# tesseract-robotics/trajopt

Hardware: NVIDIA B200
Metric: converged trajectories/sec (7-DOF x 30 wp, batch 1024) (higher is better)
Workload: dtype f64

## Files before the change

### trajopt_b200/csrc/qp_cta_kernel.cuh

```cuda
#pragma once
#include "device_types.cuh"
#include "joint_terms.cuh"

namespace tb200 {

#ifdef TB200_PROFILE
static __device__ unsigned long long g_prof[16];
#define PROF_T0() const long long prof_t0_ = clock64()
#define PROF_ADD(slot) do { if (q.tid == 0) atomicAdd(&g_prof[slot], (unsigned long long)(clock64() - prof_t0_)); } while (0)
#else
#define PROF_T0()
#define PROF_ADD(slot)
#endif
#if defined(TB200_PROFILE) && defined(TB200_PROFILE_CHECK)
#define PROF_CHK_T0() long long pc_ = clock64()
#define PROF_CHK(slot) do { const long long n_ = clock64(); if (q.tid == 0) atomicAdd(&g_prof[slot], (unsigned long long)(n_ - pc_)); pc_ = n_; } while (0)
#else
#define PROF_CHK_T0()
#define PROF_CHK(slot)
#endif

constexpr int kQpThreads = 256;
constexpr int kQpThreadsC = 256;
constexpr double kOsqpInf = 1e30;
// ... 100 lines not shown
  return s;
}

enum RowF {
  R_C = 0, R_W,
  R_E, R_DA0, R_DA1, R_EA0, R_EA1,
  R_U0, R_U1, R_B0, R_B1, R_LO, R_UP, R_QA0, R_QA1, R_RHO,
  R_XA0, R_XA1, R_Z, R_Y, R_ZA0, R_ZA1, R_YA0, R_YA1,
  R_RA0, R_RA1, R_COEF, R_WR, R_G0, R_G1, R_DEN, R_WRR,
  R_IDEN, R_IWRR,
  R_DY, R_DYA0, R_DYA1, R_DXA0, R_DXA1,
  R_PW, R_PWA0, R_PWA1, R_PB, R_PY, R_PYA0, R_PYA1, R_PX0, R_PX1,
  R_MV,
  R_NF
};
__host__ __device__ inline int qp_row_stride(int CN) { return 3 * CN + R_NF; }

struct SmVec {
  int off;
  __device__ __forceinline__ double* ptr() const {
    extern __shared__ double sm[];
    return sm + off;
  }
  __device__ __forceinline__ double& operator[](int i) const { return ptr()[i]; }
  __device__ __forceinline__ operator double*() const { return ptr(); }
  __device__ __forceinline__ SmVec& operator=(double* p) {
    extern __shared__ double sm[];
    off = static_cast<int>(p - sm);
    return *this;
  }
};

struct QpCtx {
  int N, Np, nb, M, T, D, CN, RS, tid, nrows;
  double *SA, *SLM, *SU;
  SmVec beta, x, zb, yb, v1, w, qs, lbs, ubs, tmp, red, flag;
  int* colptr;
  SmVec Dz, v2;
  double* rows;
  double* soa;
  double* smbase;
  int rows_smem;
  int* rints;
  const int* colent;
  const double* Pband;
  const int* band_offs;
  int n_band;
  double* scratch;
  int pinv;
  PinvPlan pl;
  double* pi_g;
  double* z_stash;
  double c, cinv, rho, rho_eq, sigma, alpha;
  __device__ __forceinline__ double* R(int r) const { return rows + static_cast<size_t>(r) * RS; }
  __device__ __forceinline__ double* F(int r) const { return rows + static_cast<size_t>(r) * RS + 2 * CN; }
  __device__ __forceinline__ const int* I(int r) const { return rints + static_cast<size_t>(r) * RI_NINTS; }
};

__device__ __forceinline__ double warp_max_norm(double v) {
  v = (v != v) ? 0.0 : v;
  const unsigned hi = static_cast<unsigned>(__double2hiint(v)) & 0x7fffffffu, lo = static_cast<unsigned>(__double2loint(v));
  const unsigned mh = __reduce_max_sync(0xffffffffu, hi);
  const unsigned ml = __reduce_max_sync(0xffffffffu, hi == mh ? lo : 0u);
  return __hiloint2double(static_cast<int>(mh), static_cast<int>(ml));
}
template <int NQ, unsigned SUM_MASK>
__device__ __forceinline__ void block_reduce(const QpCtx& q, double (&vals)[NQ]) {
  static_assert(NQ <= 16, "red area too small");
  extern __shared__ double sm[];
  double* const red = sm + (q.red - q.smbase);
  const int lane = q.tid & 31, wid = q.tid >> 5;
  __syncwarp();
#pragma unroll
  for (int k = 0; k < NQ; ++k) {
    double v = vals[k];
    if ((SUM_MASK >> k) & 1u) {
#pragma unroll
      for (int off = 16; off > 0; off >>= 1) v += __shfl_xor_sync(0xffffffffu, v, off);
    } else {
      v = warp_max_norm(v);
    }
    vals[k] = v;
  }
  if (lane == 0) {
#pragma unroll
    for (int k = 0; k < NQ; ++k) red[k * 8 + wid] = vals[k];
  }
  __syncthreads();
#pragma unroll
  for (int k = 0; k < NQ; ++k) {
    if ((SUM_MASK >> k) & 1u) {
      double acc = red[k * 8];
#pragma unroll
      for (int w = 1; w < kQpThreads / 32; ++w) acc += red[k * 8 + w];
      vals[k] = acc;
    } else {
      vals[k] = warp_max_norm(red[k * 8 + (lane & 7)]);
    }
  }
  __syncthreads();
}

struct SysW {
  bool polish;
  double sig, rho_aux;
};

__device__ __forceinline__ int row_var(const int* I, int k) {
  return I[RI_BASE] + min(k, I[RI_CNT] - 1) * I[RI_STRIDE];
}

template <int NB>
__device__ __forceinline__ void load_row(double (&a)[NB], const double* src) {
  const double2* s2 = reinterpret_cast<const double2*>(src);
#pragma unroll
  for (int k = 0; k < NB / 2; ++k) {
    const double2 v = s2[k];
    a[2 * k] = v.x;
    a[2 * k + 1] = v.y;
  }
}
template <int NB>
__device__ __forceinline__ void store_row(double* dst, const double (&a)[NB]) {
  double2* d2 = reinterpret_cast<double2*>(dst);
#pragma unroll
  for (int k = 0; k < NB / 2; ++k) d2[k] = make_double2(a[2 * k], a[2 * k + 1]);
}
template <int NB>
__device__ __forceinline__ void row_times_mat(double (&out)[NB], const double (&x)[NB], const double* Y) {
#pragma unroll
  for (int k = 0; k < NB; ++k) {
    double y[NB];
    load_row<NB>(y, Y + k * NB);
#pragma unroll
    for (int j = 0; j < NB; ++j) out[j] += x[k] * y[j];
  }
}
template <int NB>
__device__ __forceinline__ void row_times_matT(double (&out)[NB], const double (&x)[NB], const double* Y) {
#pragma unroll
  for (int j = 0; j < NB; ++j) {
    double y[NB];
    load_row<NB>(y, Y + j * NB);
    double a0 = 0.0, a1 = 0.0;
#pragma unroll
    for (int k = 0; k < NB; k += 2) {
      a0 += x[k] * y[k];
      a1 += x[k + 1] * y[k + 1];
    }
    out[j] += a0 + a1;
  }
}
template <int NB>
__device__ inline bool bcr_factor(const QpCtx& q) {
  constexpr int BLK = NB * NB, G = kQpThreads / 2;
  constexpr int CH1 = kQpThreads / NB, CH2 = G / NB;
  const int M = q.M, tid = q.tid;
  const int grp = tid >= G, gt = tid - (grp ? G : 0);
  int bad = 0;
  for (int l = 0; (1 << l) - 1 < M; ++l) {
    const int s = 1 << l, first = s - 1, sh = l + 1;
    const int nE = (M + s) >> sh, nS = M >> sh;
    for (int e0 = 0; e0 < nE; e0 += CH1) {
      const int nc = (nE - e0 < CH1) ? nE - e0 : CH1;
      const bool act = tid < nc * NB;
      const int e = act ? tid / NB : 0, i = tid % NB;
      double* A = q.SA + (first + ((e0 + e) << sh)) * BLK + i * NB;
      double a[NB];
      load_row<NB>(a, A);
#pragma unroll
      for (int k = 0; k < NB; ++k) {
        double* prow = q.tmp + (k & 1) * (CH1 * NB) + e * NB;
        if (act && i == k) {
          const double piv = a[k];
          if (!(piv > 0.0)) bad = 1;
          const double ip = 1.0 / piv;
#pragma unroll
          for (int j = 0; j < NB; ++j) a[j] = (j == k) ? ip : a[j] * ip;
          store_row<NB>(prow, a);
        }
        __syncthreads();
        if (act && i != k) {
          double pr[NB];
          load_row<NB>(pr, prow);
          const double f = a[k];
#pragma unroll
          for (int j = 0; j < NB; ++j) a[j] = (j == k) ? -f * pr[k] : a[j] - f * pr[j];
        }
      }
      if (act) store_row<NB>(A, a);
    }
    __syncthreads();
    for (int e0 = 0; e0 < nE; e0 += CH2) {
      const int nc = (nE - e0 < CH2) ? nE - e0 : CH2;
      const bool act = gt < nc * NB;
      const int e = e0 + (act ? gt / NB : 0), i = gt % NB;
      const int p = first + (e << sh);
      const double* Ai = q.SA + p * BLK;
      if (act && grp == 0 && p + s < M) {
        double x[NB], out[NB];
        load_row<NB>(x, q.SLM + (p + s) * BLK + i * NB);
#pragma unroll
        for (int j = 0; j < NB; ++j) out[j] = 0.0;
        row_times_mat<NB>(out, x, Ai);
        store_row<NB>(q.SU + p * BLK + i * NB, out);
      }
      if (act && grp == 1 && p - s >= 0) {
        double x[NB], out[NB];
        const double* L = q.SLM + p * BLK + i;
#pragma unroll
        for (int k = 0; k < NB; ++k) x[k] = L[k * NB];
#pragma unroll
        for (int j = 0; j < NB; ++j) out[j] = 0.0;
        row_times_mat<NB>(out, x, Ai);
        store_row<NB>(q.SU + (p - s) * BLK + i * NB, out);
      }
    }
    __syncthreads();
    for (int e0 = 0; e0 < nS; e0 += CH2) {
      const int nc = (nS - e0 < CH2) ? nS - e0 : CH2;
      const bool act = gt < nc * NB;
      const int e = e0 + (act ? gt / NB : 0), i = gt % NB;
      const int j = first + s + (e << sh), p = j - s;
      double keep[NB];
#pragma unroll
      for (int c = 0; c < NB; ++c) keep[c] = 0.0;
      if (act && grp == 0) {
        double x[NB], t1[NB];
        load_row<NB>(x, q.SU + p * BLK + i * NB);
#pragma unroll
        for (int c = 0; c < NB; ++c) t1[c] = 0.0;
        row_times_matT<NB>(t1, x, q.SLM + j * BLK);
        if (p - s >= 0) row_times_mat<NB>(keep, x, q.SLM + p * BLK);
        double arow[NB];
        load_row<NB>(arow, q.SA + j * BLK + i * NB);
#pragma unroll
        for (int c = 0; c < NB; ++c) arow[c] -= t1[c];
        store_row<NB>(q.SA + j * BLK + i * NB, arow);
      }
      if (act && grp == 1 && j + s < M) {
        double x[NB];
        load_row<NB>(x, q.SU + j * BLK + i * NB);
        row_times_mat<NB>(keep, x, q.SLM + (j + s) * BLK);
      }
      __syncthreads();
      if (act && grp == 0) {
#pragma unroll
        for (int c = 0; c < NB; ++c) keep[c] = -keep[c];
        store_row<NB>(q.SLM + j * BLK + i * NB, keep);
      }
      if (act && grp == 1 && j + s < M) {
        double arow[NB];
        load_row<NB>(arow, q.SA + j * BLK + i * NB);
#pragma unroll
        for (int c = 0; c < NB; ++c) arow[c] -= keep[c];
        store_row<NB>(q.SA + j * BLK + i * NB, arow);
      }
    }
    __syncthreads();
    for (int t = tid; t < nE * BLK; t += kQpThreads) {
      const int e = t / BLK, r = t % BLK;
      const int p = first + (e << sh);
      if (p - s >= 0) q.SLM[p * BLK + r] = q.SU[(p - s) * BLK + r];
    }
    __syncthreads();
  }
  if (tid == 0) q.flag[0] = 0.0;
  __syncthreads();
  if (bad) q.flag[0] = 1.0;
  __syncthreads();
  const bool ok = q.flag[0] == 0.0;
  __syncthreads();
  return ok;
}

template <int NB>
__device__ __forceinline__ double dot_row(const double* __restrict__ m, const double* __restrict__ v) {
  const double2* m2 = reinterpret_cast<const double2*>(m);
  const double2* v2 = reinterpret_cast<const double2*>(v);
  double a0 = 0.0, a1 = 0.0;
#pragma unroll
  for (int k = 0; k < NB / 2; ++k) {
    const double2 mm = m2[k], vv = v2[k];
    a0 += mm.x * vv.x;
    a1 += mm.y * vv.y;
  }
  return a0 + a1;
}
template <int NB>
__device__ inline void bcr_solve(const QpCtx& q, double* v, double* w) {
  constexpr int BLK = NB * NB, H = NB / 2;
  const int M = q.M, tid = q.tid, side = tid & 1, task0 = tid >> 1;
  __syncthreads();
  int l = 0;
  for (; (2 << l) - 1 < M; ++l) {
    const int s = 1 << l, sh = l + 1, nS = M >> sh;
    for (int tb = 0; tb < nS * NB; tb += kQpThreads / 2) {
      if (tb + ((tid & ~31) >> 1) >= nS * NB) continue;
      const int task = tb + task0;
      const int e = task / NB, r = task % NB;
      const bool act = e < nS;
      const int j = 2 * s - 1 + ((act ? e : 0) << sh);
      const int pb = side ? j + s : j - s;
      const bool valid = act && pb < M;
      const int pbc = valid ? pb : j - s;
      const double* mat = (side ? q.SLM : q.SU) + pbc * BLK + r * NB;
      double a = dot_row<NB>(mat, v + pbc * NB);
      a = valid ? a : 0.0;
      const double o = __shfl_xor_sync(0xffffffffu, a, 1);
      if (act && side == 0) v[j * NB + r] -= a + o;
    }
    __syncthreads();
  }
  for (; l >= 0; --l) {
    const int s = 1 << l, first = s - 1, sh = l + 1;
    if (first >= M) continue;
    const int nE = (M + s) >> sh;
    for (int tb = 0; tb < nE * NB; tb += kQpThreads / 2) {
      if (tb + ((tid & ~31) >> 1) >= nE * NB) continue;
      const int task = tb + task0;
      const int e = task / NB, r = task % NB;
      const bool act = e < nE;
      const int p = first + ((act ? e : 0) << sh);
      const bool hasl = p - s >= 0, hasr = p + s < M;
      const double* X = (side ? q.SU : q.SA) + p * BLK + r;
      const double* y = side ? w + (hasr ? p + s : 0) * NB : v + p * NB;
      const double* Um = q.SLM + p * BLK + (side ? H * NB : 0) + r;
      const double* wl = w + (hasl ? p - s : 0) * NB + (side ? H : 0);
      double a0 = 0.0, a1 = 0.0, a2 = 0.0;
#pragma unroll
      for (int k = 0; k < NB; k += 2) {
        a0 += X[k * NB] * y[k];
        a1 += X[(k + 1) * NB] * y[k + 1];
      }
#pragma unroll
      for (int k = 0; k < H; ++k) a2 += Um[k * NB] * wl[k];
      const double dx = a0 + a1;
      const double acc = (side ? (hasr ? -dx : 0.0) : dx) - (hasl ? a2 : 0.0);
      const double o = __shfl_xor_sync(0xffffffffu, acc, 1);
      if (act && side == 0) w[p * NB + r] = acc + o;
    }
    __syncthreads();
  }
}

struct SolveRoles {
  int n_fwd, n_lvl;
  int f0_warps, b0_warps;
  int f0_vec, f0_dst, b0_y, b0_wl, b0_dst;
  int fu_level, fu_vec, fu_dst, bu_level, bu_y, bu_wl, bu_dst;
  bool f0_valid, f0_store, b0_store, b0_hasl, b0_hasr, b0_yw;
  bool fu_valid, fu_store, bu_store, bu_hasl, bu_hasr, bu_yw;
  int fu_mat, bu_X, bu_Um, f0_mat, b0_X, b0_Um;
};
template <int NB>
__device__ inline SolveRoles solve_roles(const QpCtx& q) {
  SolveRoles R{};
  const int M = q.M, tid = q.tid;
  int nf = 0;
  while ((2 << nf) - 1 < M) ++nf;
  int nl = 0;
  while ((1 << nl) - 1 < M) ++nl;
  R.n_fwd = nf;
  R.n_lvl = nl;
  constexpr int BLK = NB * NB;
  const int oSA = static_cast<int>(q.SA - q.smbase), oSLM = static_cast<int>(q.SLM - q.smbase), oSU = static_cast<int>(q.SU - q.smbase);
  auto fwd_role = [&](int l, int u, int& vec, int& dst, bool& valid, bool& store) {
    const int s = 1 << l, sh = l + 1, nS = M >> sh;
    const int task = u >> 1, side = u & 1, e = task / NB, r = task % NB;
    const bool act = e < nS;
    const int j = 2 * s - 1 + ((act ? e : 0) << sh);
    const int pb = side ? j + s : j - s;
    valid = act && pb < M;
    vec = (valid ? pb : j - s) * NB;
    dst = j * NB + r;
    store = act && side == 0;
    (l > 0 ? R.fu_mat : R.f0_mat) = (side ? oSLM : oSU) + (valid ? pb : j - s) * BLK + r * NB;
  };
  auto bwd_role = [&](int l, int u, int& y, int& wl, int& dst, bool& store, bool& hasl, bool& hasr, bool& yw) {
    const int s = 1 << l, first = s - 1, sh = l + 1, nE = (M + s) >> sh;
    const int task = u >> 1, side = u & 1, e = task / NB, r = task % NB;
    const bool act = e < nE;
    const int p = first + ((act ? e : 0) << sh);
    hasl = p - s >= 0;
    hasr = p + s < M;
    yw = side;
    y = side ? (hasr ? p + s : 0) * NB : p * NB;
    wl = (hasl ? p - s : 0) * NB + (side ? NB / 2 : 0);
    dst = p * NB + r;
    store = act && side == 0;
    (l > 0 ? R.bu_X : R.b0_X) = (side ? oSU : oSA) + p * BLK + r;
    (l > 0 ? R.bu_Um : R.b0_Um) = oSLM + p * BLK + (side ? (NB / 2) * NB : 0) + r;
  };
  fwd_role(0, tid, R.f0_vec, R.f0_dst, R.f0_valid, R.f0_store);
  R.f0_warps = (2 * (M >> 1) * NB + 31) & ~31;
  bwd_role(0, tid, R.b0_y, R.b0_wl, R.b0_dst, R.b0_store, R.b0_hasl, R.b0_hasr, R.b0_yw);
  R.b0_warps = (2 * ((M + 1) >> 1) * NB + 31) & ~31;
  R.fu_level = -1;
  R.bu_level = -1;
  int off = 0;
  for (int l = 1; l < nf; ++l) {
    const int cnt = 2 * (M >> (l + 1)) * NB;
    if (tid >= off && tid < off + cnt) {
      R.fu_level = l;
      fwd_role(l, tid - off, R.fu_vec, R.fu_dst, R.fu_valid, R.fu_store);
    }
    off += cnt;
  }
  off = 0;
  for (int l = 1; l < nl; ++l) {
    const int cnt = 2 * ((M + (1 << l)) >> (l + 1)) * NB;
    if (tid >= off && tid < off + cnt) {
      R.bu_level = l;
      bwd_role(l, tid - off, R.bu_y, R.bu_wl, R.bu_dst, R.bu_store, R.bu_hasl, R.bu_hasr, R.bu_yw);
    }
    off += cnt;
  }
  return R;
}
__host__ __device__ inline bool solve_roles_fit(int M, int NB) {
  int f = 0, b = 0;
  for (int l = 1; (2 << l) - 1 < M; ++l) f += 2 * (M >> (l + 1)) * NB;
  for (int l = 1; (1 << l) - 1 < M; ++l) b += 2 * ((M + (1 << l)) >> (l + 1)) * NB;
  return f <= kQpThreads && b <= kQpThreads && 2 * ((M + 1) >> 1) * NB <= kQpThreads;
}
template <int NB>
// ... 259 lines not shown
  __syncthreads();
  for (int l = 1; l < R.n_fwd; ++l) {
    const bool mine = R.fu_level == l;
    if (__any_sync(0xffffffffu, mine)) {
      double a = reg_fwd_task<NB>(mFU, v + (mine ? R.fu_vec : 0));
      a = (mine && R.fu_valid) ? a : 0.0;
      const double o = __shfl_xor_sync(0xffffffffu, a, 1);
      if (mine && R.fu_store) v[R.fu_dst] -= a + o;
    }
    __syncthreads();
  }
  for (int l = R.n_lvl - 1; l >= 1; --l) {
    const bool mine = R.bu_level == l;
    if (__any_sync(0xffffffffu, mine)) {
      double acc = reg_bwd_task<NB>(mBU, (R.bu_yw ? w : v) + (mine ? R.bu_y : 0), w + (mine ? R.bu_wl : 0), R.bu_yw,
                                    R.bu_hasl, R.bu_hasr);
      acc = mine ? acc : 0.0;
      const double o = __shfl_xor_sync(0xffffffffu, acc, 1);
      if (mine && R.bu_store) w[R.bu_dst] = acc + o;
    }
    __syncthreads();
  }
  if (wbase < R.b0_warps) {
    const double acc = reg_bwd_task<NB>(mB0, (side ? w : v) + R.b0_y, w + R.b0_wl, side, R.b0_hasl, R.b0_hasr);
    const double o = __shfl_xor_sync(0xffffffffu, acc, 1);
    if (R.b0_store) w[R.b0_dst] = acc + o;
  }
  __syncthreads();
}

template <int NB>
__device__ __forceinline__ void bcr_solve_hyb(const int tid, const SolveRoles& R, const double (&mF0)[NB],
                                              const double (&mB0)[NB + NB / 2], const double* sm_base, double* v, double* w) {
  const int wbase = tid & ~31;
  const bool side = tid & 1;
  __syncthreads();
  if (wbase < R.f0_warps) {
#ifndef TB200_HYB_F0_REGS
    double a = bcr_fwd_task<NB>(sm_base + R.f0_mat, v + R.f0_vec);
#else
    double a = reg_fwd_task<NB>(mF0, v + R.f0_vec);
#endif
    a = R.f0_valid ? a : 0.0;
    const double o = __shfl_xor_sync(0xffffffffu, a, 1);
    if (R.f0_store) v[R.f0_dst] -= a + o;
  }
  __syncthreads();
  for (int l = 1; l < R.n_fwd; ++l) {
    const bool mine = R.fu_level == l;
    if (__any_sync(0xffffffffu, mine)) {
      double a = bcr_fwd_task<NB>(sm_base + (mine ? R.fu_mat : 0), v + (mine ? R.fu_vec : 0));
      a = (mine && R.fu_valid) ? a : 0.0;
      const double o = __shfl_xor_sync(0xffffffffu, a, 1);
      if (mine && R.fu_store) v[R.fu_dst] -= a + o;
    }
    __syncthreads();
  }
  for (int l = R.n_lvl - 1; l >= 1; --l) {
    const bool mine = R.bu_level == l;
    if (__any_sync(0xffffffffu, mine)) {
      double acc = bcr_bwd_task<NB>(sm_base + (mine ? R.bu_X : 0), sm_base + (mine ? R.bu_Um : 0),
                                    (R.bu_yw ? w : v) + (mine ? R.bu_y : 0), w + (mine ? R.bu_wl : 0), R.bu_yw, R.bu_hasl,
                                    R.bu_hasr);
      acc = mine ? acc : 0.0;
      const double o = __shfl_xor_sync(0xffffffffu, acc, 1);
      if (mine && R.bu_store) w[R.bu_dst] = acc + o;
    }
    __syncthreads();
  }
  if (wbase < R.b0_warps) {
    const double acc = reg_bwd_task<NB>(mB0, (side ? w : v) + R.b0_y, w + R.b0_wl, side, R.b0_hasl, R.b0_hasr);
    const double o = __shfl_xor_sync(0xffffffffu, acc, 1);
    if (R.b0_store) w[R.b0_dst] = acc + o;
  }
  __syncthreads();
}

template <int NB>
__device__ __forceinline__ void p_matvec(const QpCtx& q, const double* in, double* out) {
  extern __shared__ double sm[];
  constexpr int HB = NB, W = HB + 1;
  const int N = q.N, Np = q.Np, nbo = q.n_band;
  const double* const Pb = q.Pband;
  const double* const Dz = sm + (q.Dz - q.smbase);
  const double* const vin = sm + (in - q.smbase);
  double* const vout = sm + (out - q.smbase);
  const int* const offs = q.band_offs;
  const double cc = q.c;
  for (int i = q.tid; i < Np; i += kQpThreads) {
    double s = 0.0;
    if (i < N) {
      for (int t0 = 0; t0 < nbo; t0 += 4) {
        double v[4];
#pragma unroll
        for (int u = 0; u < 4; ++u) {
          const int k = (t0 + u < nbo) ? offs[t0 + u] : -1;
          v[u] = (k >= 0 && k <= i) ? (Pb[i * W + k] * Dz[i - k]) * vin[i - k] : 0.0;
        }
        s += v[0]; s += v[1]; s += v[2]; s += v[3];
      }
      for (int t0 = 0; t0 < nbo; t0 += 4) {
        double v[4];
#pragma unroll
        for (int u = 0; u < 4; ++u) {
          const int k = (t0 + u < nbo) ? offs[t0 + u] : -1;
          v[u] = (k >= 1 && i + k < N) ? (Pb[(i + k) * W + k] * Dz[i + k]) * vin[i + k] : 0.0;
        }
        s += v[0]; s += v[1]; s += v[2]; s += v[3];
      }
      s *= cc * Dz[i];
    }
    vout[i] = s;
  }
  __syncthreads();
}

__device__ inline void rows_prepare_weights(const QpCtx& q, const SysW& w) {
  for (int r = q.tid; r < q.nrows; r += kQpThreads) {
    double* F = q.F(r);
    const int naux = q.I(r)[RI_AUX];
    const double Wr = w.polish ? fabs(F[R_PW]) : ((F[R_RHO] != 0.0) ? q.rho_eq : q.rho);
    const double wa0 = w.polish ? fabs(F[R_PWA0]) : w.rho_aux;
    const double wa1 = w.polish ? fabs(F[R_PWA1]) : w.rho_aux;
    const double g0 = (naux >= 1) ? w.sig + wa0 * F[R_B0] * F[R_B0] : 1.0;
    const double g1 = (naux == 2) ? w.sig + wa1 * F[R_B1] * F[R_B1] : 1.0;
    const double den = g0 * g1 + Wr * (F[R_U0] * F[R_U0] * g1 + F[R_U1] * F[R_U1] * g0);
    F[R_WRR] = Wr;
    F[R_G0] = g0;
    F[R_G1] = g1;
    F[R_DEN] = den;
    F[R_IDEN] = 1.0 / den;
    F[R_IWRR] = (Wr != 0.0) ? 1.0 / Wr : 0.0;
    F[R_WR] = Wr * g0 * g1 / den;
  }
  __syncthreads();
}
__device__ __forceinline__ double xbound_weight(const QpCtx& q, const SysW& w, int j) {
  const double adm = (q.ubs[j] - q.lbs[j] < kRhoTol) ? q.rho_eq : q.rho;
  return w.polish ? fabs(q.zb[j]) : adm;
}

__device__ __forceinline__ double pivot_rcp(const double x) {
  double r;
  asm("rcp.approx.ftz.f64 %0, %1;" : "=d"(r) : "d"(x));
  double e = fma(-x, r, 1.0);
  r = fma(r, e, r);
  e = fma(-x, r, 1.0);
  r = fma(r, e, r);
  e = fma(-x, r, 1.0);
  return fma(r, e, r);
}
template <int QN>
__device__ __forceinline__ bool gj_rows(double (&a)[QN], double diag, const bool active, const int mat, const int row,
                                        const int n, const int n_max, double* tmp, const int nmat) {
  constexpr int BS = QN + 2;
  double* const csv = tmp + 2 * nmat * BS + mat * QN;
  bool bad = false;
  double pv_mine = pivot_rcp(diag), my_cs = 1.0, rs = 1.0, inv_rs = 1.0;
#pragma unroll 1
  for (int k = 0; k < n_max; ++k) {
    double* buf = tmp + ((k & 1) * nmat + mat) * BS;
    const bool piv = active && row == k;
    if (piv) {
      bad |= !(diag > 0.0);
#pragma unroll
      for (int j = 0; j < QN; j += 2) *reinterpret_cast<double2*>(buf + j) = make_double2(a[j], a[j + 1]);
      buf[k] = 0.0;
      buf[QN] = pv_mine;
      my_cs = -pv_mine;
      csv[k] = my_cs;
      rs = pv_mine;
      inv_rs = diag;
      diag = pv_mine;
    }
    __syncthreads();
    if (active && k < n && !piv) {
      const double tr = buf[row];
      const bool ahead = row > k;
      const double f = ahead ? tr : -tr * my_cs;
      const double g = f * buf[QN];
      diag = ahead ? diag - g * f : diag + g * f;
      const double gs = g * inv_rs;
#pragma unroll
      for (int j = 0; j < QN; j += 2) {
        const double2 t = *reinterpret_cast<const double2*>(buf + j);
        a[j] -= gs * t.x;
        a[j + 1] -= gs * t.y;
      }
      if (ahead) pv_mine = pivot_rcp(diag);
    }
  }
  if (active) {
#pragma unroll
    for (int j = 0; j < QN; ++j) a[j] = (j == row) ? diag : ((j < n) ? a[j] * (rs * csv[j]) : 0.0);
  }
  return bad;
}

template <int NB>
__device__ inline bool pinv_factor(const QpCtx& q) {
  constexpr int QN = 3 * NB, blk = NB * NB;
  static_assert(QN % 2 == 0, "pivot rows move as double2");
  extern __shared__ double sm[];
  const int tid = q.tid, M = q.M, Np = q.Np;
  const int PR = q.pl.PR, nS = q.pl.nS, Ns = q.pl.Ns, ZS = q.pl.ZS, WS = q.pl.WS, SS = q.pl.SS;
  double* const fbase = sm + (q.SA - q.smbase);
  const double* const SA = fbase;
  const double* const SLM = sm + (q.SLM - q.smbase);
  double* const Z = fbase + q.pl.zo;
  double* const W = fbase + q.pl.wo;
  double* const S = fbase + q.pl.so;
  double* const tmp = q.tmp.ptr();
  const int nparts = (M + 3) / 4;
  bool bad = false;
#ifdef TB200_PROFILE
  long long pf_ = clock64();
#define PROF_PF(slot) do { const long long n_ = clock64(); if (tid == 0) atomicAdd(&g_prof[slot], (unsigned long long)(n_ - pf_)); pf_ = n_; } while (0)
#else
#define PROF_PF(slot)
#endif
  {
    const bool prow = tid < PR;
    const int p = prow ? tid / QN : 0, lr = prow ? tid % QN : 0;
    const int npb = (M - 4 * p) < 3 ? (M - 4 * p) : 3;
    const int kb = lr / NB, r = lr % NB, gb = 4 * p + kb;
    double a[QN];
#pragma unroll
    for (int j = 0; j < QN; ++j) {
      const int cb = j / NB, c = j % NB;
      double v = 0.0;
      if (prow && cb < npb) {
        if (cb == kb) v = SA[gb * blk + r * NB + c];
        else if (cb == kb - 1) v = SLM[gb * blk + r * NB + c];
        else if (cb == kb + 1) v = SLM[(gb + 1) * blk + c * NB + r];
      }
      a[j] = v;
    }
    PROF_PF(0);
    const double dg = prow ? SA[gb * blk + r * NB + r] : 1.0;
    bad |= gj_rows<QN>(a, dg, prow, p, lr, npb * NB, (M < 3 ? M : 3) * NB, tmp, nparts);
    PROF_PF(4);
    if (prow) {
#pragma unroll
      for (int j = 0; j < QN; ++j) q.pi_g[tid * QN + j] = a[j];
      const bool has_l = p > 0, has_r = 4 * p + 3 < M;
#pragma unroll 2
      for (int j = 0; j < NB; ++j) {
        double wl = 0.0, wr = 0.0;
        if (has_l) {
#pragma unroll
          for (int c = 0; c < NB; ++c) wl += a[c] * SLM[(4 * p) * blk + c * NB + j];
        }
        if (has_r) {
#pragma unroll
          for (int c = 0; c < NB; ++c) wr += a[2 * NB + c] * SLM[(4 * p + 3) * blk + j * NB + c];
        }
        W[tid * WS + j] = wl;
        W[tid * WS + NB + j] = wr;
      }
    }
  }
  __syncthreads();
  for (int e = tid; e < nS * nS; e += kQpThreads) {
    const int ra = e / nS, ca = e % nS, sa = ra / NB, i = ra % NB, sb = ca / NB, j = ca % NB;
    double v = 0.0;
    if (sa == sb || sb == sa + 1 || sb == sa - 1) {
      const bool use_l = sb <= sa, use_r = sb >= sa && 4 * sa + 4 < M;
      const double* cl = SLM + (4 * sa + 3) * blk + i * NB;
      const double* wl = W + (sa * QN + 2 * NB) * WS + (sb == sa ? NB : 0) + j;
      const double* cr = SLM + (4 * sa + 4) * blk + i;
      const double* wr = W + ((sa + 1) * QN) * WS + (sb == sa ? 0 : NB) + j;
      double s0 = 0.0, s1 = 0.0, s2 = 0.0, s3 = 0.0;
      if (use_l) {
#pragma unroll
        for (int rr = 0; rr < NB; rr += 2) {
          s0 += cl[rr] * wl[rr * WS];
          s1 += cl[rr + 1] * wl[(rr + 1) * WS];
        }
      }
      if (use_r) {
#pragma unroll
        for (int rr = 0; rr < NB; rr += 2) {
          s2 += cr[rr * NB] * wr[rr * WS];
          s3 += cr[(rr + 1) * NB] * wr[(rr + 1) * WS];
        }
      }
      v = ((sa == sb) ? SA[(4 * sa + 3) * blk + i * NB + j] : 0.0) - ((s0 + s1) + (s2 + s3));
    }
    S[ra * SS + ca] = v;
  }
  __syncthreads();
  PROF_PF(14);
  {
    const bool srow = tid < nS;
    double a[QN];
#pragma unroll
    for (int j = 0; j < QN; ++j) a[j] = (srow && j < nS) ? S[tid * SS + j] : 0.0;
    const double dg = srow ? S[tid * SS + tid] : 1.0;
    bad |= gj_rows<QN>(a, dg, srow, 0, tid, nS, nS, tmp, 1);
    if (srow) {
#pragma unroll
      for (int j = 0; j < QN; ++j)
        if (j < nS) S[tid * SS + j] = a[j];
    }
  }
  __syncthreads();
  PROF_PF(15);
  if (tid < Np) {
    const int col = tid, cb = col / NB, c = col % NB, p = cb / 4;
    if (cb % 4 == 3) {
      for (int sr = 0; sr < nS; ++sr) Z[sr * ZS + col] = S[sr * SS + p * NB + c];
    } else {
      const bool has_l = p > 0, has_r = 4 * p + 3 < M;
      const double* wrow = W + (p * QN + (cb % 4) * NB + c) * WS;
      double wv[2 * NB];
#pragma unroll
      for (int t = 0; t < 2 * NB; ++t) wv[t] = wrow[t];
      const double* sl = S + (has_l ? (p - 1) * NB : 0);
      const double* sr_ = S + (has_r ? p * NB : 0);
#pragma unroll 2
      for (int sr = 0; sr < nS; ++sr) {
        double s0 = 0.0, s1 = 0.0, s2 = 0.0, s3 = 0.0;
#pragma unroll
        for (int t = 0; t < NB; t += 2) {
          s0 += sl[sr * SS + t] * wv[t];
          s1 += sl[sr * SS + t + 1] * wv[t + 1];
          s2 += sr_[sr * SS + t] * wv[NB + t];
          s3 += sr_[sr * SS + t + 1] * wv[NB + t + 1];
        }
        Z[sr * ZS + col] = -((s0 + s1) + (s2 + s3));
      }
    }
  }
  (void)Ns;
  const bool ok = !__syncthreads_or(bad ? 1 : 0);
  PROF_PF(9);
  return ok;
}

template <int NB, bool PINV>
__device__ __noinline__ bool assemble_factor(const QpCtx& q, const SysW& w) {
  PROF_T0();
  rows_prepare_weights(q, w);
  constexpr int nb = NB, blk = NB * NB;
  const int N = q.N, HB = 2 * q.D, PW = HB + 1, CN = q.CN;
  for (int t = q.tid; t < q.M * blk; t += kQpThreads) {
    q.SA[t] = 0.0;
    q.SLM[t] = 0.0;
  }
  __syncthreads();
  for (int i = q.tid; i < q.Np; i += kQpThreads) {
    const int p = i / nb, r = i % nb;
    double* Arow = q.SA + static_cast<size_t>(p) * blk + r * nb;
    double* Lrow = q.SLM + static_cast<size_t>(p) * blk + r * nb;
    if (i >= N) {
      Arow[r] = 1.0;
      continue;
    }
    auto add = [&](int k, double val) {
      if (k <= r) Arow[r - k] += val;
      else Lrow[nb + r - k] += val;
    };
    for (int t = 0; t < q.n_band; ++t) {
      const int k = q.band_offs[t];
      if (k <= i) add(k, q.c * q.Dz[i] * q.Pband[i * PW + k] * q.Dz[i - k]);
    }
    add(0, w.sig + xbound_weight(q, w, i) * q.beta[i] * q.beta[i]);
    for (int e = q.colptr[i]; e < q.colptr[i + 1]; ++e) {
      const int ent = q.colent[e], rw = ent >> 5, k = ent & 31;
      const double* R = q.R(rw);
      const double wr = R[2 * CN + R_WR];
      if (wr == 0.0) continue;
      const int stride = q.I(rw)[RI_STRIDE];
      const double* as = R + CN;
      const double ai = wr * as[k];
      for (int k2 = 0; k2 <= k; ++k2) add((k - k2) * stride, ai * as[k2]);
    }
  }
  __syncthreads();
  for (int t = q.tid; t < q.M * blk; t += kQpThreads) {
    const int p = t / blk, i = (t % blk) / nb, j = t % nb;
    if (j > i) q.SA[static_cast<size_t>(p) * blk + i * nb + j] = q.SA[static_cast<size_t>(p) * blk + j * nb + i];
  }
  __syncthreads();
  PROF_ADD(10);
  bool ok;
  {
    PROF_T0();
    if constexpr (PINV) ok = pinv_factor<NB>(q);
    else ok = bcr_factor<NB>(q);
    PROF_ADD(11);
  }
  return ok;
}

struct QpOut {
  int status, iters, polish;
  double rho;
  double pri_res, dua_res, pol_pri, pol_dua, c;
  int pol_factor_ok, rho_updates, rounds;
};

template <int CN, class Base>
__device__ __forceinline__ void scatter_columns(const QpCtx& q, Base base) {
  for (int i = q.tid; i < q.Np; i += kQpThreads) {
    double s = 0.0;
    if (i < q.N) {
      s = base(i);
      for (int e = q.colptr[i]; e < q.colptr[i + 1]; ++e) {
        const int ent = q.colent[e], r = ent >> 5, k = ent & 31;
        const double* R = q.R(r);
        s += R[CN + k] * R[2 * CN + R_COEF];
      }
    }
    q.v1[i] = s;
  }
  __syncthreads();
}
template <int CN>
__device__ __forceinline__ double row_dot(const QpCtx& q, const double* R, const int* I, const double* v) {
  double z = 0.0;
  const int base = I[RI_BASE], stride = I[RI_STRIDE], last = I[RI_CNT] - 1;
#pragma unroll
  for (int k = 0; k < CN; ++k) z += R[CN + k] * v[base + min(k, last) * stride];
  return z;
}
__device__ __forceinline__ void row_backsub(const double* F, double zeta, double& a0, double& a1) {
  const double Wr = F[R_WRR], ra0 = F[R_RA0], ra1 = F[R_RA1], u0 = F[R_U0], u1 = F[R_U1];
  const double iden = F[R_IDEN];
  a0 = (F[R_G1] * (ra0 - Wr * u0 * zeta) + Wr * u1 * (u1 * ra0 - u0 * ra1)) * iden;
  a1 = (F[R_G0] * (ra1 - Wr * u1 * zeta) + Wr * u0 * (u0 * ra1 - u1 * ra0)) * iden;
}
__device__ __forceinline__ double row_reduce_coef(const double* F, double ra0, double ra1, double zcoef) {
  return zcoef - F[R_WRR] * (F[R_U0] * ra0 * F[R_G1] + F[R_U1] * ra1 * F[R_G0]) * F[R_IDEN];
}

template <int NB, int PAIR, bool REG>
__device__ __noinline__ void admm_block(const QpCtx& q, const double rho_aux, const int n_iter, const int keep_last) {
  constexpr int CNc = PAIR ? ((NB > 3) ? NB : 3) : ((NB / 2 > 3) ? NB / 2 : 3);
  constexpr int RNB = REG ? NB : 2;
  const int N = q.N, tid = q.tid;
  double* const dxs = q.scratch;
  double* const dyb = q.scratch + q.Np;
  SolveRoles roles{};
  double mF0[RNB], mB0[RNB + RNB / 2], mFU[RNB], mBU[RNB + RNB / 2];
  if constexpr (REG) {
    roles = solve_roles<NB>(q);
    load_fwd_row<NB>(q, 0, tid, mF0);
    load_bwd_row<NB>(q, 0, tid, mB0);
    int off = 0;
    for (int l = 1; l < roles.n_fwd; ++l) {
      const int cnt = 2 * (q.M >> (l + 1)) * NB;
// ... 1752 lines not shown
```

Before: 1485.

## Use warp-per-block BCR factorization and named barriers in pinv Gauss-Jordan

Adds a warp-level block cyclic reduction factor path for NB<=16, where each warp factors one diagonal block with __syncwarp instead of CTA-wide barriers. The pinv partition Gauss-Jordan now gives each partition two warps and syncs them with per-partition named barriers, so independent partitions do not wait on each other. The loop bound drops to each partition's own size, and the reciprocal pivot is computed only for the next pivot row. The change risks named-barrier ID limits, a reduced thread count when nparts*64 exceeds the block, and lower parallelism inside each block factor.

```diff
diff --git a/trajopt_b200/csrc/qp_cta_kernel.cuh b/trajopt_b200/csrc/qp_cta_kernel.cuh
--- a/trajopt_b200/csrc/qp_cta_kernel.cuh
+++ b/trajopt_b200/csrc/qp_cta_kernel.cuh
@@ -276,7 +276,113 @@
   }
 }
 template <int NB>
-__device__ inline bool bcr_factor(const QpCtx& q) {
+__device__ __forceinline__ bool bcr_factor_warp(const QpCtx& q) {
+  static_assert(NB <= 16, "two row groups per warp");
+  constexpr int BLK = NB * NB, NW = kQpThreads / 32;
+  const int M = q.M, lane = q.tid & 31, warp = q.tid >> 5;
+  const int grp = lane >> 4, i = lane & 15;
+  const bool act = i < NB, gj = lane < NB;
+  double* const pbuf = q.tmp + warp * (2 * NB);
+  int bad = 0;
+  for (int l = 0; (1 << l) - 1 < M; ++l) {
+    const int s = 1 << l, first = s - 1, sh = l + 1;
+    const int nE = (M + s) >> sh, nS = M >> sh;
+    for (int e = warp; e < nE; e += NW) {
+      const int p = first + (e << sh);
+      double* const A = q.SA + p * BLK;
+      double a[NB];
+      load_row<NB>(a, A + (gj ? lane : 0) * NB);
+#pragma unroll
+      for (int k = 0; k < NB; ++k) {
+        double* prow = pbuf + (k & 1) * NB;
+        if (lane == k) {
+          const double piv = a[k];
+          if (!(piv > 0.0)) bad = 1;
+          const double ip = 1.0 / piv;
+#pragma unroll
+          for (int j = 0; j < NB; ++j) a[j] = (j == k) ? ip : a[j] * ip;
+          store_row<NB>(prow, a);
+        }
+        __syncwarp();
+        if (gj && lane != k) {
+          double pr[NB];
+          load_row<NB>(pr, prow);
+          const double f = a[k];
+#pragma unroll
+          for (int j = 0; j < NB; ++j) a[j] = (j == k) ? -f * pr[k] : a[j] - f * pr[j];
+        }
+      }
+      if (gj) store_row<NB>(A + lane * NB, a);
+      __syncwarp();
+      if (act && grp == 0 && p + s < M) {
+        double x[NB], out[NB];
+        load_row<NB>(x, q.SLM + (p + s) * BLK + i * NB);
+#pragma unroll
+        for (int j = 0; j < NB; ++j) out[j] = 0.0;
+        row_times_mat<NB>(out, x, A);
+        store_row<NB>(q.SU + p * BLK + i * NB, out);
+      }
+      if (act && grp == 1 && p - s >= 0) {
+        double x[NB], out[NB];
+        const double* L = q.SLM + p * BLK + i;
+#pragma unroll
+        for (int k = 0; k < NB; ++k) x[k] = L[k * NB];
+#pragma unroll
+        for (int j = 0; j < NB; ++j) out[j] = 0.0;
+        row_times_mat<NB>(out, x, A);
+        store_row<NB>(q.SU + (p - s) * BLK + i * NB, out);
+      }
+    }
+    __syncthreads();
+    for (int e = warp; e < nS; e += NW) {
+      const int j = first + s + (e << sh), p = j - s;
+      double keep[NB];
+#pragma unroll
+      for (int c = 0; c < NB; ++c) keep[c] = 0.0;
+      if (act && grp == 0) {
+        double x[NB], t1[NB];
+        load_row<NB>(x, q.SU + p * BLK + i * NB);
+#pragma unroll
+        for (int c = 0; c < NB; ++c) t1[c] = 0.0;
+        row_times_matT<NB>(t1, x, q.SLM + j * BLK);
+        if (p - s >= 0) row_times_mat<NB>(keep, x, q.SLM + p * BLK);
+        double arow[NB];
+        load_row<NB>(arow, q.SA + j * BLK + i * NB);
+#pragma unroll
+        for (int c = 0; c < NB; ++c) arow[c] -= t1[c];
+        store_row<NB>(q.SA + j * BLK + i * NB, arow);
+      }
+      if (act && grp == 1 && j + s < M) {
+        double x[NB];
+        load_row<NB>(x, q.SU + j * BLK + i * NB);
+        row_times_mat<NB>(keep, x, q.SLM + (j + s) * BLK);
+      }
+      __syncwarp();
+      if (act && grp == 0) {
+#pragma unroll
+        for (int c = 0; c < NB; ++c) keep[c] = -keep[c];
+        store_row<NB>(q.SLM + j * BLK + i * NB, keep);
+      }
+      if (act && grp == 1 && j + s < M) {
+        double arow[NB];
+        load_row<NB>(arow, q.SA + j * BLK + i * NB);
+#pragma unroll
+        for (int c = 0; c < NB; ++c) arow[c] -= keep[c];
+        store_row<NB>(q.SA + j * BLK + i * NB, arow);
+      }
+    }
+    __syncthreads();
+    for (int t = q.tid; t < nE * BLK; t += kQpThreads) {
+      const int e = t / BLK, r = t % BLK;
+      const int p = first + (e << sh);
+      if (p - s >= 0) q.SLM[p * BLK + r] = q.SU[(p - s) * BLK + r];
+    }
+    __syncthreads();
+  }
+  return !__syncthreads_or(bad);
+}
+template <int NB>
+__device__ inline bool bcr_factor_cta(const QpCtx& q) {
   constexpr int BLK = NB * NB, G = kQpThreads / 2;
   constexpr int CH1 = kQpThreads / NB, CH2 = G / NB;
   const int M = q.M, tid = q.tid;
@@ -396,6 +502,11 @@
   const bool ok = q.flag[0] == 0.0;
   __syncthreads();
   return ok;
+}
+template <int NB>
+__device__ __forceinline__ bool bcr_factor(const QpCtx& q) {
+  if constexpr (NB <= 16) return bcr_factor_warp<NB>(q);
+  else return bcr_factor_cta<NB>(q);
 }
 
 template <int NB>
@@ -961,13 +1072,13 @@
 }
 template <int QN>
 __device__ __forceinline__ bool gj_rows(double (&a)[QN], double diag, const bool active, const int mat, const int row,
-                                        const int n, const int n_max, double* tmp, const int nmat) {
+                                        const int n, double* tmp, const int nmat, const int bar_id, const int bar_n) {
   constexpr int BS = QN + 2;
   double* const csv = tmp + 2 * nmat * BS + mat * QN;
   bool bad = false;
   double pv_mine = pivot_rcp(diag), my_cs = 1.0, rs = 1.0, inv_rs = 1.0;
 #pragma unroll 1
-  for (int k = 0; k < n_max; ++k) {
+  for (int k = 0; k < n; ++k) {
     double* buf = tmp + ((k & 1) * nmat + mat) * BS;
     const bool piv = active && row == k;
     if (piv) {
@@ -982,8 +1093,8 @@
       inv_rs = diag;
       diag = pv_mine;
     }
-    __syncthreads();
-    if (active && k < n && !piv) {
+    asm volatile("bar.sync %0, %1;" ::"r"(bar_id), "r"(bar_n) : "memory");
+    if (active && !piv) {
       const double tr = buf[row];
       const bool ahead = row > k;
       const double f = ahead ? tr : -tr * my_cs;
@@ -996,7 +1107,7 @@
         a[j] -= gs * t.x;
         a[j + 1] -= gs * t.y;
       }
-      if (ahead) pv_mine = pivot_rcp(diag);
+      if (row == k + 1) pv_mine = pivot_rcp(diag);
     }
   }
   if (active) {
@@ -1012,7 +1123,7 @@
   static_assert(QN % 2 == 0, "pivot rows move as double2");
   extern __shared__ double sm[];
   const int tid = q.tid, M = q.M, Np = q.Np;
-  const int PR = q.pl.PR, nS = q.pl.nS, Ns = q.pl.Ns, ZS = q.pl.ZS, WS = q.pl.WS, SS = q.pl.SS;
+  const int nS = q.pl.nS, Ns = q.pl.Ns, ZS = q.pl.ZS, WS = q.pl.WS, SS = q.pl.SS;
   double* const fbase = sm + (q.SA - q.smbase);
   const double* const SA = fbase;
   const double* const SLM = sm + (q.SLM - q.smbase);
@@ -1028,10 +1139,12 @@
 #else
 #define PROF_PF(slot)
 #endif
-  {
-    const bool prow = tid < PR;
-    const int p = prow ? tid / QN : 0, lr = prow ? tid % QN : 0;
+  static_assert(QN <= 64, "a partition's rows fit its two warps");
+  if (tid >> 6 < nparts) {
+    const int p = tid >> 6, lr0 = tid & 63;
     const int npb = (M - 4 * p) < 3 ? (M - 4 * p) : 3;
+    const bool prow = lr0 < npb * NB;
+    const int lr = prow ? lr0 : 0, row = p * QN + lr;
     const int kb = lr / NB, r = lr % NB, gb = 4 * p + kb;
     double a[QN];
 #pragma unroll
@@ -1047,11 +1160,11 @@
     }
     PROF_PF(0);
     const double dg = prow ? SA[gb * blk + r * NB + r] : 1.0;
-    bad |= gj_rows<QN>(a, dg, prow, p, lr, npb * NB, (M < 3 ? M : 3) * NB, tmp, nparts);
+    bad |= gj_rows<QN>(a, dg, prow, p, lr, npb * NB, tmp, nparts, 1 + p, 64);
     PROF_PF(4);
     if (prow) {
 #pragma unroll
-      for (int j = 0; j < QN; ++j) q.pi_g[tid * QN + j] = a[j];
+      for (int j = 0; j < QN; ++j) q.pi_g[row * QN + j] = a[j];
       const bool has_l = p > 0, has_r = 4 * p + 3 < M;
 #pragma unroll 2
       for (int j = 0; j < NB; ++j) {
@@ -1064,8 +1177,8 @@
 #pragma unroll
           for (int c = 0; c < NB; ++c) wr += a[2 * NB + c] * SLM[(4 * p + 3) * blk + j * NB + c];
         }
-        W[tid * WS + j] = wl;
-        W[tid * WS + NB + j] = wr;
+        W[row * WS + j] = wl;
+        W[row * WS + NB + j] = wr;
       }
     }
   }
@@ -1100,13 +1213,13 @@
   }
   __syncthreads();
   PROF_PF(14);
-  {
+  if (tid < 64) {
     const bool srow = tid < nS;
     double a[QN];
 #pragma unroll
     for (int j = 0; j < QN; ++j) a[j] = (srow && j < nS) ? S[tid * SS + j] : 0.0;
     const double dg = srow ? S[tid * SS + tid] : 1.0;
-    bad |= gj_rows<QN>(a, dg, srow, 0, tid, nS, nS, tmp, 1);
+    bad |= gj_rows<QN>(a, dg, srow, 0, tid, nS, tmp, 1, 1, 64);
     if (srow) {
 #pragma unroll
       for (int j = 0; j < QN; ++j)
```

New measurement: 1477, median of 6. No clear change (-0.5%).
